# GEOS-ESM/GEOSradiation_GridComp

Measured on AMD Instinct MI355X. Metric: columns/sec (LW+SW, 72 layers), higher is better.
Workload: dtype f32; 1 GPU; BASELINE configs[3] (C360 tile / 8 GPUs) per-GPU share: 97200 columns/GPU, 72 layers, RRTMG_LW (140 g-points) + RRTMG_SW (112 g-points), McICA clouds on 60 % of the columns (ih=1), aerosols on, every column lit; schemes=RRTMG_LW (140 g-points) + RRTMG_SW (112 g-points), columns_per_gpu=97200, layers=72, aerosol=True, hip_streams=2

## Files before the change

geosradiation_gridcomp_amd/csrc/geosrad.hip:

```cpp
#include <hip/hip_runtime.h>

#include <cstdio>
#include <cstdlib>
#include <cstring>
#include <map>
#include <string>
#include <tuple>
#include <vector>
#include <thread>
#include <mutex>
#include <condition_variable>
#include <memory>
#include <atomic>
#include <functional>
#include <chrono>

#include <dlfcn.h>
#include <sched.h>
#include <cstddef>
#include <cstdint>
#include "../../include/geosrad.h"
#include "../../include/geosrad_gettau.h"
#include "../../include/geosrad_satsim.h"
#include "../../include/geosrad_misr_modis.h"
// ... 728 lines not shown
static inline ArrShape ic_in_shape(int k, size_t L) { return {k == geosrad_ctx::IC_PHALF ? L + 1 : k == geosrad_ctx::IC_SKT ? 1 : L, 1}; }
static inline ArrShape ic_out_shape(int k, size_t S) { return {k == geosrad_ctx::ICO_FQ ? 49 : k >= geosrad_ctx::ICO_BOXTAU ? S : 1, 1}; }
static inline ArrShape modis_in_shape(int k, size_t L, size_t S) { return {k == geosrad_ctx::MDI_PH ? L + 1 : k >= geosrad_ctx::MDI_BOXTAU ? S : L, 1}; }
static inline ArrShape modis_out_shape(int k, size_t S) { return {k == geosrad_ctx::MDO_MEAN ? (size_t)17 : k == geosrad_ctx::MDO_HIST ? (size_t)49 : S, 1}; }
static inline ArrShape misr_out_shape(int k) { return {k == geosrad_ctx::MIO_FQ ? (size_t)(7 * 16) : k == geosrad_ctx::MIO_DIST ? (size_t)16 : (size_t)1, 1}; }

struct HostArrs {
    size_t E;
    std::vector<geosrad_ctx::PipeArr> arrs;
    std::vector<const void **> at;
    explicit HostArrs(size_t real_bytes) : E(real_bytes) {}
    void add(const void *src, void *dst, ArrShape s, const void **at_, size_t ebytes = 0)
    {
        arrs.push_back({src, dst, s.rows, s.rec * (ebytes ? ebytes : E), 0});
        at.push_back(at_);
    }
    void add(const void *src, void *dst, ArrShape s, void **at_, size_t ebytes = 0) { add(src, dst, s, (const void **)at_, ebytes); }
    void add_clear_counts(int32_t *dst, void **at_) { add(nullptr, dst, {4, 1}, at_, sizeof(int32_t)); }
};

geosrad_ctx *geosrad_new_ctx_f32();
geosrad_ctx *geosrad_new_ctx_f64();

#if !defined(GEOSRAD_PART) || GEOSRAD_PART != 0
namespace {

#define LAUNCH_WIDE(kernel, wide, ncol, rows, st, arg) do {                                                            \
        if (wide) hipLaunchKernelGGL((kernel<R, VW>), dim3(grid256((ncol) / VW), rows), dim3(256), 0, st, arg);       \
        else hipLaunchKernelGGL((kernel<R, 1>), dim3(grid256(ncol), rows), dim3(256), 0, st, arg); } while (0)
template <typename R> struct Ctx : geosrad_ctx {
    using R2 = typename Vec2<R>::T;
    DevBuf<> d_tab, d_xcw;
    size_t so_lds_set = 0;
    LwDev<R> h_T{};
    DevBuf<LwDev<R>> d_T;
    bool have_lw = false;
    DevBuf<> d_tab_sw;
    SwDev<R> h_S{};
    std::vector<R> avgcyc_mg, avgcyc_sb;
    DevBuf<SwDev<R>> d_S;
    bool have_sw = false;
    DevBuf<> d_ws_sw; int ws_sw_ncol = 0, ws_sw_nlay = 0, ws_sw_planes = 0; bool ws_sw_radval = false;
    DevBuf<> d_tab_so;
    SoradDev<R> h_O{};
    DevBuf<SoradDev<R>> d_O;
    bool have_sorad = false;
// ... 287 lines not shown
        if constexpr (SW) {
            hipLaunchKernelGGL(k_sw_validate<R>, dim3(gx), blk, 0, st, A);
        } else hipLaunchKernelGGL(k_validate_pwv<R>, dim3(gx), blk, 0, st, A, d_T);
        launch_partition(st, A.ncol, A.colcloudy, A.perm, A.nclear);
        span_end(st);
        span_begin(SW ? 7 : 1, st);
        if constexpr (SW) hipLaunchKernelGGL(k_sw_setcoef<R>, dim3(gx, A.nlay), blk, 0, st, A, dS);
        else hipLaunchKernelGGL((k_setcoef<R, true>), dim3(gx, A.nlay), blk, 0, st, A, d_T);
        span_end(st);
        span_begin(2, st);
        hipLaunchKernelGGL(k_overlap<R>, dim3(gx, A.nlay), blk, 0, st, A.ncol, A.ld, A.nlay, A.doy, A.zm, A.alat, (const int32_t *)A.perm,
                           (const int32_t *)A.nclear, dT, A.alpha, A.rcorr, A.laycloudy);
        span_end(st);
        McArgs<R> M{};
        M.ncol = A.ncol; M.ld = A.ld; M.nlay = A.nlay; M.nsubcol = SW ? NG_SW : NG_LW; M.doy = A.doy; M.cloudLM = A.cloudLM; M.cloudMH = A.cloudMH;
        M.iceflg = A.iceflg; M.liqflg = A.liqflg;
        for (int k = 0; k < 4; k++) M.so[k] = SW ? 4 - k : 1 + k;
        M.cwp_tiny = (R)1.e-20;
        M.play = A.play; M.ciwp = A.ciwp; M.clwp = A.clwp; M.rei = A.rei; M.rel = A.rel;
        M.alpha = A.alpha; M.rcorr = A.rcorr; M.perm = A.perm; M.nclear = A.nclear; M.cftop = A.colcloudy;
        M.taucmc = A.taucmc; M.laycloudy = A.laycloudy; M.clearCounts = A.clearCounts; M.err = A.err;
        if constexpr (SW) { M.cldf = A.cld; M.ssacmc = A.ssacmc; M.asmcmc = A.asmcmc; M.cotsum = A.cotsum; M.rvsum = rvsum; }
        else M.cldf = A.cldf;
        McPlan MP; int nseg = 0;
        if (const int rc = mc_plan(MODE, M.nsubcol, A.nlay, MP, nseg)) return rc;
        const dim3 grid(xcd_grid(A.ncol, 64, nseg));
        span_begin(3, st);
        if constexpr (SW) {
            if (radval) hipLaunchKernelGGL((k_mcica<R, 2, true>), grid, dim3(64), 0, st, M, MP, dT, dS);
            else hipLaunchKernelGGL((k_mcica<R, 2>), grid, dim3(64), 0, st, M, MP, dT, dS);
        } else hipLaunchKernelGGL((k_mcica<R, 0>), grid, dim3(64), 0, st, M, MP, dT, dS);
        span_end(st);
        return GEOSRAD_OK;
    }

    int lw_sweeps(hipStream_t st, const LwArgs<R> &A, const LwOut<R> &O, bool allow_cols)
    {
        const dim3 blk(256);
        const unsigned gx = grid256(A.ncol);
        const size_t lds = lw_bands_lds_bytes<R>();
        const bool cols = lw_cols_path && allow_cols;
        LwArgs<R> S = A;
        if (O.part_alt) S.part = const_cast<R *>(O.part_alt);
        span_begin(4, st);
        if (cols) {
            if (const int rc = hip_rc("lw_cols_launch", lw_cols_launch<R>(st, S, O, h_T, A.dbg_taug != nullptr))) return rc;
// ... 957 lines not shown
    size_t ws_layout_sw(int nc, int nlay, SwArgs<R> &w, R *&rvsum, Carve c, int planes, bool radval) const
    {
        const size_t cl = (size_t)nlay * nc;
        w.sc = c.take<R>(SW_NFIELD * cl);
        w.scidx = c.take<uint32_t>(cl);
        w.colcloudy = c.take<uint8_t>(nc);
        w.perm = c.take<int32_t>(nc);
        w.nclear = c.take<int32_t>(1 + part_blocks(nc));
        w.laycloudy = c.take<uint8_t>(cl);
        w.alpha = c.take<R>(cl);
        w.rcorr = c.take<R>(cl);
        w.taucmc = c.take<R>(NG_SW * cl);
        w.ssacmc = c.take<R>(NG_SW * cl);
        w.asmcmc = c.take<R>(NG_SW * cl);
        w.cotsum = c.take<R>((size_t)3 * NG_SW * nc);
        w.cell = c.take<R>((size_t)planes * NG_SW * nlay * (((size_t)nc + 255) & ~(size_t)255));
        const size_t slots = sw_path == 2 ? (size_t)(sw_reform_nslot<R>() > NB_SW ? sw_reform_nslot<R>() : NB_SW) : (size_t)NB_SW;
        w.part = c.take<R>((size_t)4 * slots * (nlay + 1) * nc);
        w.bsfc = c.take<R>((size_t)3 * slots * nc);
        w.cot = c.take<R>((size_t)8 * 6 * nc);
        rvsum = radval ? c.take<R>((size_t)3 * RV_NSUM * RV_NPAR * nc) : nullptr;
        return c.off;
    }
    int sw_planes(bool dbg) const { return (sw_path == 2 && !dbg) ? (sizeof(R) == 4 ? 5 : 15) : 14; }
    int ensure_ws_sw(int nc, int nlay, int planes, bool radval)
    {
        if (d_ws_sw && nc <= ws_sw_ncol && nlay == ws_sw_nlay && planes <= ws_sw_planes && (ws_sw_radval || !radval)) return GEOSRAD_OK;
        if (planes < ws_sw_planes) planes = ws_sw_planes;
        radval = radval || ws_sw_radval;
        const int want = (d_ws_sw && nlay == ws_sw_nlay && nc < ws_sw_ncol) ? ws_sw_ncol : nc;
        SwArgs<R> w; R *rvsum;
        const size_t need = ws_layout_sw(want, nlay, w, rvsum, Carve(), planes, radval);
        if (d_ws_sw.resize(need) != hipSuccess) return fail(GEOSRAD_ENOMEM, "hipMalloc of the SW workspace failed (" + std::to_string(need >> 20) +
                                                         " MiB); lower it with geosrad_set_chunk()");
        ws_sw_ncol = want; ws_sw_nlay = nlay; ws_sw_planes = planes; ws_sw_radval = radval;
        return GEOSRAD_OK;
    }

    static bool nrl_adjust(R solcycfr, const R *indsolvar, R *scl)
    {
        const R fmin = (R)0.0189, fmax = (R)0.3750, dmin2max = fmax - fmin, dmax2min = (R)1. - dmin2max;
        if (solcycfr >= 0 && solcycfr < fmin) {
            const R wgt = (solcycfr + (R)1. - fmax) / dmax2min;
            scl[0] = indsolvar[0] + wgt * ((R)1. - indsolvar[0]); scl[1] = indsolvar[1] + wgt * ((R)1. - indsolvar[1]);
        } else if (solcycfr >= fmin && solcycfr <= fmax) {
            const R wgt = (solcycfr - fmin) / dmin2max;
            scl[0] = (R)1. + wgt * (indsolvar[0] - (R)1.); scl[1] = (R)1. + wgt * (indsolvar[1] - (R)1.);
// ... 134 lines not shown
        return GEOSRAD_OK;
    }
    int sw_check_arrays(const void *const *in, void *const *out, int iaer, int do_drfband)
    {
        for (int k = 0; k < S_NIN; k++)
            if (!in[k] && !((k == S_TAUAER || k == S_SSAAER || k == S_ASMAER) && iaer != 10)) return fail(GEOSRAD_EINVAL, "null input array");
        for (int k = 0; k < SO_DRBAND; k++) if (!out[k]) return fail(GEOSRAD_EINVAL, "null output array");
        if (do_drfband && (!out[SO_DRBAND] || !out[SO_DFBAND])) return fail(GEOSRAD_EINVAL, "do_drfband set but drband/dfband null");
        return GEOSRAD_OK;
    }

    int sw_run(hipStream_t st, int ncol, int nlay, double scon, double adjes, int isolvar, const void *const *in, int iceflg, int liqflg,
               int dyofyr, int iaer, int cloudLM, int cloudMH, int normFlx, int32_t *clearCounts, void *const *out, int do_drfband,
               const void *bndscl, const void *indsolvar, const void *solcycfrac, void *const *dbg, void *const *sw_na_out,
               void *radval = nullptr)
    {
        HIPCHK(hipSetDevice(device));
        if (const int rc = sw_check_options(ncol, nlay, iceflg, liqflg, cloudLM, cloudMH, iaer)) return rc;
        if (const int rc = sw_check_arrays(in, out, iaer, do_drfband)) return rc;
        if (radval && dbg) return fail(GEOSRAD_EINVAL, "the stage dumps do not produce the SOLAR_RADVAL diagnostics");
        SwSolar<R> SV;
        if (const int rc = sw_solar(scon, adjes, isolvar, (const R *)bndscl, (const R *)indsolvar, (const R *)solcycfrac, SV)) return rc;

        const int nc_max = chunk_cols(ncol, (long)(0xFFFFFFFFull / ((unsigned long long)nlay * 12ull * sizeof(R))) & ~255L);
        if (const int rc = ensure_ws_sw(nc_max, nlay, sw_planes(dbg != nullptr), radval != nullptr)) return rc;

        return chunk_walk(ncol, nc_max, [&](int c0, int nc) -> int {
            SwArgs<R> A{};
            R *rvsum;
            ws_layout_sw(nc, nlay, A, rvsum, Carve(d_ws_sw), ws_sw_planes, ws_sw_radval);
            A.ncol = nc; A.ld = ncol; A.nlay = nlay; A.iceflg = iceflg; A.liqflg = liqflg; A.doy = dyofyr; A.cloudLM = cloudLM;
            A.cloudMH = cloudMH; A.iaer = iaer; A.normFlx = normFlx; A.do_drfband = do_drfband;
            auto P = [&](int k) { return colp(in[k], c0); };
            A.play = P(S_PLAY); A.plev = P(S_PLEV); A.tlay = P(S_TLAY); A.h2o = P(S_H2O); A.o3 = P(S_O3); A.co2 = P(S_CO2);
            A.ch4 = P(S_CH4); A.o2 = P(S_O2); A.cld = P(S_CLD); A.ciwp = P(S_CIWP); A.clwp = P(S_CLWP); A.rei = P(S_REI);
            A.rel = P(S_REL); A.zm = P(S_ZM); A.alat = P(S_ALAT);
            A.tauaer = iaer == 10 ? P(S_TAUAER) : nullptr; A.ssaaer = iaer == 10 ? P(S_SSAAER) : nullptr;
            A.asmaer = iaer == 10 ? P(S_ASMAER) : nullptr;
            A.coszen = P(S_COSZEN); A.asdir = P(S_ASDIR); A.asdif = P(S_ASDIF); A.aldir = P(S_ALDIR); A.aldif = P(S_ALDIF);
            A.err = d_err + 1;
            A.clearCounts = clearCounts + c0;
            const size_t d0 = (size_t)c0 * NG_SW * nlay;
            if (dbg) { A.dbg_taug = (R *)dbg[0] + d0; A.dbg_taur = (R *)dbg[1] + d0; A.dbg_ssi = (R *)dbg[2] + (size_t)c0 * NG_SW; }
            if (const int e = rrtmg_front<2>(st, A, radval != nullptr, rvsum)) return e;
            const dim3 blk(256);
            const unsigned gx = grid256(nc);
            if (radval) {
// ... 1788 lines not shown

static __global__ void k_dbg_fast64(int n, const double *__restrict__ a, const double *__restrict__ b, double *__restrict__ q,
                                    double *__restrict__ r, double *__restrict__ s)
{
    const int i = blockIdx.x * blockDim.x + threadIdx.x;
    if (i < n) { q[i] = geosrad::gr_div64(a[i], b[i]); r[i] = geosrad::gr_rcp64(b[i]); s[i] = geosrad::gr_sqrt64(b[i]); }
}
int geosrad_dbg_fast64(int n, const double *a, const double *b, double *quot, double *rcp, double *root)
{
    if (n <= 0 || !a || !b || !quot || !rcp || !root) return GEOSRAD_EINVAL;
    DevBuf<double> d;
    const size_t nb = (size_t)n * sizeof(double);
    if (d.resize(5 * nb) != hipSuccess) return GEOSRAD_EHIP;
    int rc = GEOSRAD_OK;
    if (hipMemcpy(d, a, nb, hipMemcpyHostToDevice) != hipSuccess || hipMemcpy(d + n, b, nb, hipMemcpyHostToDevice) != hipSuccess) rc = GEOSRAD_EHIP;
    if (rc == GEOSRAD_OK) {
        k_dbg_fast64<<<(n + 255) / 256, 256>>>(n, d, d + n, d + 2 * (size_t)n, d + 3 * (size_t)n, d + 4 * (size_t)n);
        if (hipMemcpy(quot, d + 2 * (size_t)n, nb, hipMemcpyDeviceToHost) != hipSuccess || hipMemcpy(rcp, d + 3 * (size_t)n, nb, hipMemcpyDeviceToHost) != hipSuccess ||
            hipMemcpy(root, d + 4 * (size_t)n, nb, hipMemcpyDeviceToHost) != hipSuccess) rc = GEOSRAD_EHIP;
    }
    return rc;
}

int geosrad_rrtmg_lw_taumol(geosrad_ctx *c, int ncol, int nlay, const void *play, const void *plev, const void *tlay, const void *tlev,
                            const void *tsfc, const void *emis, const void *h2ovmr, const void *o3vmr, const void *co2vmr,
                            const void *ch4vmr, const void *n2ovmr, const void *o2vmr, const void *cfc11vmr, const void *cfc12vmr,
                            const void *cfc22vmr, const void *ccl4vmr, const void *tauaer, void *taug, void *pfracs)
{
    if (!c || !taug || !pfracs) return GEOSRAD_EINVAL;
    const size_t esz = (size_t)c->real_kind;
    std::vector<char> zero((size_t)ncol * (nlay + 1) * esz, 0), ones((size_t)ncol * nlay * esz, 0), scratch((size_t)ncol * (nlay + 1) * esz * 4);
    for (size_t i = 0; i < (size_t)ncol * nlay; i++) { if (esz == 4) ((float *)ones.data())[i] = 10.f; else ((double *)ones.data())[i] = 10.; }
    std::vector<int32_t> cc((size_t)ncol * 4);
    const void *cldf = zero.data(), *ciwp = zero.data(), *clwp = zero.data(), *rei = ones.data(), *rel = ones.data(), *zm = zero.data(),
               *alat = zero.data();
    LW_PACK_IN();
    char *s = scratch.data();
    const size_t cv = (size_t)ncol * (nlay + 1) * esz;
    void *out[O_NOUT] = {s, s + cv, s + 2 * cv, s + 3 * cv, nullptr, nullptr, nullptr, nullptr};
    return c->lw_host(ncol, nlay, 0, in, 3, 1, 1, 1, 2, cc.data(), out, nullptr, taug, pfracs);
}

int geosrad_mcica(geosrad_ctx *c, int ncol, int nsubcol, int nlay, const void *zmid, const void *alat, int doy, const void *play,
                  const void *cldfrac, const void *ciwp, const void *clwp, double cwp_tiny, const int32_t seed_order[4],
                  int32_t *cldy_stoch, void *ciwp_stoch, void *clwp_stoch)
{
// ... 36 lines not shown
```

geosradiation_gridcomp_amd/csrc/lw_kernels.hpp:

```cpp
#pragma once
#include "lw_device.hpp"
#include <type_traits>

namespace geosrad {

#define GR_DEV __device__ __forceinline__

template <typename R> GR_DEV R gr_exp(R x);
template <> GR_DEV float gr_exp<float>(float x) { return expf(x); }
template <> GR_DEV double gr_exp<double>(double x) { return exp(x); }
template <typename R> GR_DEV R gr_log(R x);
template <> GR_DEV float gr_log<float>(float x) { return logf(x); }
template <> GR_DEV double gr_log<double>(double x) { return log(x); }
template <typename R> GR_DEV R gr_log10(R x);
template <> GR_DEV float gr_log10<float>(float x) { return log10f(x); }
template <> GR_DEV double gr_log10<double>(double x) { return log10(x); }
template <typename R> GR_DEV R gr_pow(R x, R y);
template <> GR_DEV float gr_pow<float>(float x, float y) { return powf(x, y); }
template <> GR_DEV double gr_pow<double>(double x, double y) { return pow(x, y); }

#ifndef GR_FAST64
#define GR_FAST64 1
#endif
GR_DEV double gr_rcp64(double b)
// ... 21 lines not shown
    if (x == 0.0) return 0.0;
    const double y = __builtin_amdgcn_rsq(x);
    double g = x * y, h = 0.5 * y;
    const double r = fma(-h, g, 0.5);
    g = fma(g, r, g); h = fma(h, r, h);
    g = fma(fma(-g, g, x), h, g);
    return fma(fma(-g, g, x), h, g);
#else
    return sqrt(x);
#endif
}

GR_DEV int clampi(int v, int lo, int hi) { return v < lo ? lo : (v > hi ? hi : v); }

constexpr int pad4(int n) { return (n + 3) & ~3; }

template <typename T> GR_DEV T ldg(const T *base, uint32_t byteoff)
{
    return *reinterpret_cast<const T *>(reinterpret_cast<const char *>(base) + byteoff);
}
template <typename T> GR_DEV void stg(T *base, uint32_t byteoff, T v)
{
    *reinterpret_cast<T *>(reinterpret_cast<char *>(base) + byteoff) = v;
}
template <typename T> GR_DEV T ldg_nt(const T *base, uint32_t byteoff)
{
    return __builtin_nontemporal_load(reinterpret_cast<const T *>(reinterpret_cast<const char *>(base) + byteoff));
}
template <typename T> GR_DEV void stg_nt(T *base, uint32_t byteoff, T v)
{
    __builtin_nontemporal_store(v, reinterpret_cast<T *>(reinterpret_cast<char *>(base) + byteoff));
}
GR_DEV void err_wave(bool bad, uint32_t *err, int bit)
{
    if (__ballot(bad) != 0) {
        if (bad) atomicOr(err, 1u << bit);
    }
}
typedef float gr_v2f __attribute__((ext_vector_type(2)));
typedef double gr_v2d __attribute__((ext_vector_type(2)));
template <> GR_DEV float2 ldg_nt<float2>(const float2 *base, uint32_t byteoff)
{
    const gr_v2f t = __builtin_nontemporal_load(reinterpret_cast<const gr_v2f *>(reinterpret_cast<const char *>(base) + byteoff));
    float2 r; r.x = t.x; r.y = t.y; return r;
}
template <> GR_DEV double2 ldg_nt<double2>(const double2 *base, uint32_t byteoff)
// ... 1255 lines not shown
        BAND::template prep<R>(T, A, L, P);
#pragma unroll
        for (int q = 0; q < NQ; q++) {
            R tau[W], pf[W];
            BAND::template eval<R, W>(T, L, P, q * W, tau, pf);
#pragma unroll
            for (int j = 0; j < W; j++) {
                const int g = q * W + j;
                if (g >= NG) continue;
                if (lay == 0) {
                    const R rad0 = pf[j] * plankbnd;
                    rad[g] = rad0 + reflect * rad[g];
                    dlu[g] = pf[j] * dplankbnd;
                    u0 = u0 + sumfac * rad[g];
                    du0 = du0 + sumfac * dlu[g];
                    if (CLD) {
                        radc[g] = rad0 + reflect * radc[g];
                        dclu[g] = dlu[g];
                        uc0 = uc0 + sumfac * radc[g];
                        duc0 = duc0 + sumfac * dclu[g];
                    }
                }
                const R2 e1 = lut_at((int)sv[g]);
                const R a1 = (R)1. - e1.x, b1 = pf[j] * (blay + e1.y * dplankup);
                rad[g] = rad[g] + (b1 - rad[g]) * a1;
                dlu[g] = dlu[g] - dlu[g] * a1;
                usum = usum + sumfac * rad[g];
                dusum = dusum + sumfac * dlu[g];
                if (CLD) {
                    const R2 e2 = lut_at(own ? (int)sg[g] : (int)sv[g]);
                    const R gx = (R)1. - e2.x, gy = pf[j] * (blay + e2.y * dplankup);
                    const R rc = radc[g] + (gy - radc[g]) * gx, dc = dclu[g] - dclu[g] * gx;
                    radc[g] = diverge ? rc : rad[g];
                    dclu[g] = diverge ? dc : dlu[g];
                    ucsum = ucsum + sumfac * radc[g];
                    ducsum = ducsum + sumfac * dclu[g];
                }
            }
        }
        if (lay == 0) {
            PART(2, 0, u0);
            if (CLD && ccol) PART(3, 0, uc0);
            if (dudTs) { PART(4, 0, du0); if (CLD && ccol) PART(5, 0, duc0); }
        }
        PART(2, lay + 1, usum);
        if (CLD && ccol) PART(3, lay + 1, ucsum);
        if (dudTs) { PART(4, lay + 1, dusum); if (CLD && ccol) PART(5, lay + 1, ducsum); }
    }
#undef PART
}

__constant__ const int LW_BAND_ORDER[NB_LW] = {3, 5, 4, 7, 9, 2, 1, 8, 12, 6, 11, 13, 10, 15, 16, 14};
__host__ __device__ constexpr int lw_band_g0(int ib)
{
// ... 140 lines not shown
```

geosradiation_gridcomp_amd/csrc/sw_kernels.hpp:

```cpp
#pragma once
#include "lw_kernels.hpp"

namespace geosrad {

constexpr int NB_SW = 14;
constexpr int NG_SW = 112;

enum SwGas { G_H2O = 0, G_CO2, G_O3, G_CH4, G_O2, G_NONE };
enum SwScField {
    SW_FAC00 = 0, SW_FAC01, SW_FAC10, SW_FAC11, SW_COLH2O, SW_COLCO2, SW_COLO3, SW_COLCH4, SW_COLO2, SW_COLMOL,
    SW_SELFFAC, SW_SELFFRAC, SW_FORFAC, SW_FORFRAC, SW_NFIELD
};

template <typename R> struct SwBandTab {
    const R *absa, *absb, *selfref, *forref;
    const R *sflux, *irrad, *facb, *snsp;
    const R *rayl;
    const R *x0, *x1;
    const R *raylb;
};

template <typename R> struct SwDev {
    SwBandTab<R> b[NB_SW + 1];
    const R *preflog, *tref;
// ... 120 lines not shown
    A.scidx[(size_t)lay * n + col] = pack_idx(jp, jt, jt1, indfor, indself, 0, lower ? 1 : 0);
}

struct SwB16 { static constexpr int JB = 16, NG = 6,  G0 = 0,   LOK = 2, LOA = G_H2O, LOB = G_CH4, UPK = 1, UPA = G_CH4, UPB = G_NONE, NFOR = 3, SRC = 0, LREF = 0,  NSRC = 1; static constexpr double STR = 252.131;    static constexpr bool LOCONT = true,  UPFOR = false; };
struct SwB17 { static constexpr int JB = 17, NG = 12, G0 = 6,   LOK = 2, LOA = G_H2O, LOB = G_CO2, UPK = 2, UPA = G_H2O, UPB = G_CO2,  NFOR = 4, SRC = 2, LREF = 30, NSRC = 5; static constexpr double STR = 0.364641;   static constexpr bool LOCONT = true,  UPFOR = true;  };
struct SwB18 { static constexpr int JB = 18, NG = 8,  G0 = 18,  LOK = 2, LOA = G_H2O, LOB = G_CH4, UPK = 1, UPA = G_CH4, UPB = G_NONE, NFOR = 3, SRC = 1, LREF = 6,  NSRC = 9; static constexpr double STR = 38.9589;    static constexpr bool LOCONT = true,  UPFOR = false; };
struct SwB19 { static constexpr int JB = 19, NG = 8,  G0 = 26,  LOK = 2, LOA = G_H2O, LOB = G_CO2, UPK = 1, UPA = G_CO2, UPB = G_NONE, NFOR = 3, SRC = 1, LREF = 3,  NSRC = 9; static constexpr double STR = 5.49281;    static constexpr bool LOCONT = true,  UPFOR = false; };
struct SwB20 { static constexpr int JB = 20, NG = 10, G0 = 34,  LOK = 1, LOA = G_H2O, LOB = G_NONE, UPK = 1, UPA = G_H2O, UPB = G_NONE, NFOR = 4, SRC = 0, LREF = 0,  NSRC = 1; static constexpr double STR = 0;          static constexpr bool LOCONT = true,  UPFOR = true;  };
struct SwB21 { static constexpr int JB = 21, NG = 10, G0 = 44,  LOK = 2, LOA = G_H2O, LOB = G_CO2, UPK = 2, UPA = G_H2O, UPB = G_CO2,  NFOR = 4, SRC = 1, LREF = 8,  NSRC = 9; static constexpr double STR = 0.0045321;  static constexpr bool LOCONT = true,  UPFOR = true;  };
struct SwB22 { static constexpr int JB = 22, NG = 2,  G0 = 54,  LOK = 2, LOA = G_H2O, LOB = G_O2,  UPK = 1, UPA = G_O2,  UPB = G_NONE, NFOR = 3, SRC = 1, LREF = 2,  NSRC = 9; static constexpr double STR = 1.6 * 0.022708; static constexpr bool LOCONT = true, UPFOR = false; };
struct SwB23 { static constexpr int JB = 23, NG = 10, G0 = 56,  LOK = 1, LOA = G_H2O, LOB = G_NONE, UPK = 0, UPA = G_NONE, UPB = G_NONE, NFOR = 3, SRC = 0, LREF = 0,  NSRC = 1; static constexpr double STR = 0;          static constexpr bool LOCONT = true,  UPFOR = false; };
struct SwB24 { static constexpr int JB = 24, NG = 8,  G0 = 66,  LOK = 2, LOA = G_H2O, LOB = G_O2,  UPK = 1, UPA = G_O2,  UPB = G_NONE, NFOR = 3, SRC = 1, LREF = 1,  NSRC = 9; static constexpr double STR = 0.124692;   static constexpr bool LOCONT = true,  UPFOR = false; };
struct SwB25 { static constexpr int JB = 25, NG = 6,  G0 = 74,  LOK = 1, LOA = G_H2O, LOB = G_NONE, UPK = 0, UPA = G_NONE, UPB = G_NONE, NFOR = 0, SRC = 0, LREF = 0,  NSRC = 1; static constexpr double STR = 0;          static constexpr bool LOCONT = false, UPFOR = false; };
struct SwB26 { static constexpr int JB = 26, NG = 6,  G0 = 80,  LOK = 0, LOA = G_NONE, LOB = G_NONE, UPK = 0, UPA = G_NONE, UPB = G_NONE, NFOR = 0, SRC = 0, LREF = 0,  NSRC = 1; static constexpr double STR = 0;         static constexpr bool LOCONT = false, UPFOR = false; };
struct SwB27 { static constexpr int JB = 27, NG = 8,  G0 = 86,  LOK = 1, LOA = G_O3,  LOB = G_NONE, UPK = 1, UPA = G_O3,  UPB = G_NONE, NFOR = 0, SRC = 0, LREF = 0,  NSRC = 1; static constexpr double STR = 0;          static constexpr bool LOCONT = false, UPFOR = false; };
struct SwB28 { static constexpr int JB = 28, NG = 6,  G0 = 94,  LOK = 2, LOA = G_O3,  LOB = G_O2,  UPK = 2, UPA = G_O3,  UPB = G_O2,   NFOR = 0, SRC = 2, LREF = 42, NSRC = 5; static constexpr double STR = 6.67029e-07; static constexpr bool LOCONT = false, UPFOR = false; };
struct SwB29 { static constexpr int JB = 29, NG = 12, G0 = 100, LOK = 1, LOA = G_H2O, LOB = G_NONE, UPK = 1, UPA = G_CO2, UPB = G_NONE, NFOR = 4, SRC = 0, LREF = 0,  NSRC = 1; static constexpr double STR = 0;          static constexpr bool LOCONT = true,  UPFOR = false; };

template <typename R> struct SwLayer {
    R fac00, fac01, fac10, fac11, col[5], colmol, selffac, selffrac, forfac, forfrac;
    int jp, jt, jt1, indfor, indself;
    bool lower;
};
template <typename R> GR_DEV void sw_load_layer(const SwArgs<R> &A, int lay, int col, SwLayer<R> &L)
{
    const uint32_t cell = (uint32_t)lay * (uint32_t)A.ncol + (uint32_t)col;
    const uint32_t wb = cell * (uint32_t)sizeof(R);
    const size_t fs = (size_t)A.nlay * A.ncol;
#define SCF(f) ldg(A.sc + (size_t)(f) * fs, wb)
    L.fac00 = SCF(SW_FAC00); L.fac01 = SCF(SW_FAC01); L.fac10 = SCF(SW_FAC10); L.fac11 = SCF(SW_FAC11);
    L.col[G_H2O] = SCF(SW_COLH2O); L.col[G_CO2] = SCF(SW_COLCO2); L.col[G_O3] = SCF(SW_COLO3); L.col[G_CH4] = SCF(SW_COLCH4);
    L.col[G_O2] = SCF(SW_COLO2); L.colmol = SCF(SW_COLMOL);
    L.selffac = SCF(SW_SELFFAC); L.selffrac = SCF(SW_SELFFRAC); L.forfac = SCF(SW_FORFAC); L.forfrac = SCF(SW_FORFRAC);
#undef SCF
    const uint32_t p = ldg(A.scidx, cell * 4u);
    L.jp = p & 63; L.jt = (p >> 6) & 7; L.jt1 = (p >> 9) & 7; L.indfor = (p >> 12) & 3; L.indself = (p >> 14) & 15;
    L.lower = (p >> 23) & 1;
}

template <typename R> struct SwSpec { R speccomb, fs; int js; };
template <typename R> GR_DEV SwSpec<R> sw_spec(R cola, R strrat, R colb, R mult, R oneminus)
{
    SwSpec<R> s;
    s.speccomb = cola + strrat * colb;
    R specparm = cola / s.speccomb;
    if (specparm >= oneminus) specparm = oneminus;
    const R sm = mult * specparm;
    const int j = (int)sm;
    s.js = 1 + j;
    s.fs = sm - (R)j;
    return s;
}

template <typename R> struct SwPrep { SwSpec<R> sp; int ind0, ind1; R cmaj, extra; };

template <typename R, typename B> GR_DEV void sw_prep(const SwDev<R> &T, const SwLayer<R> &L, SwPrep<R> &P)
{
    P.extra = 0; P.cmaj = 0; P.ind0 = 1; P.ind1 = 1; P.sp.fs = 0; P.sp.js = 1; P.sp.speccomb = 0;
    if (L.lower) {
        if constexpr (B::LOK == 2) {
            P.sp = sw_spec<R>(L.col[B::LOA], (R)B::STR, L.col[B::LOB], 8, T.oneminus);
// ... 690 lines not shown
```

geosradiation_gridcomp_amd/csrc/sw_reform.hip:

```cpp
#include "sw_reform_kernels.hpp"
#include "sw_reform.hpp"

namespace geosrad {

template <typename R> hipError_t sw_reform_launch(hipStream_t st, const SwArgs<R> &A, const SwDev<R> &T, const SwSolar<R> &SV)
{
    static_assert(swr_nslot<R> <= SWR_SLOTS_MAX && swr_ncot<R> <= 6, "workspace slots");
    const dim3 grid(band_grid(A.ncol, swr_nslot<R>)), blk(256);
    hipLaunchKernelGGL((k_sw_reform<R, false>), grid, blk, 0, st, A, T, SV);
    hipLaunchKernelGGL((k_sw_reform<R, true>), grid, blk, 0, st, A, T, SV);
    return hipGetLastError();
}

template <typename R> int sw_reform_nslot() { return swr_nslot<R>; }

template <typename R> int sw_reform_par_units(int *sizes)
{
    int k = 0;
    for (int jb = 24; jb <= 26; jb++)
        for (int u = 0; u < swr_nunit(swr_u<R>, sw_band_ng(jb)); u++) sizes[k++] = swr_usize(swr_u<R>, sw_band_ng(jb), u);
    return k;
}

template <typename R> hipError_t sw_reform_reduce(hipStream_t st, const SwArgs<R> &A, const SwOut<R> &O)
{
    hipLaunchKernelGGL(k_swr_reduce<R>, dim3((unsigned)((A.ncol + 255) / 256), A.nlay + 2), dim3(256), 0, st, A, O);
    return hipGetLastError();
}

#if !defined(GEOSRAD_PART) || GEOSRAD_PART == 4
template hipError_t sw_reform_launch<float>(hipStream_t, const SwArgs<float> &, const SwDev<float> &, const SwSolar<float> &);
template hipError_t sw_reform_reduce<float>(hipStream_t, const SwArgs<float> &, const SwOut<float> &);
template int sw_reform_nslot<float>();
template int sw_reform_par_units<float>(int *);
#endif
#if !defined(GEOSRAD_PART) || GEOSRAD_PART == 8
template hipError_t sw_reform_launch<double>(hipStream_t, const SwArgs<double> &, const SwDev<double> &, const SwSolar<double> &);
template hipError_t sw_reform_reduce<double>(hipStream_t, const SwArgs<double> &, const SwOut<double> &);
template int sw_reform_nslot<double>();
template int sw_reform_par_units<double>(int *);
#endif

}
```

geosradiation_gridcomp_amd/csrc/sw_reform.hpp:

```cpp
#pragma once
#include "sw_kernels.hpp"

namespace geosrad {
constexpr int SWR_SLOTS_MAX = 32;
template <typename R> int sw_reform_nslot();
template <typename R> int sw_reform_par_units(int *sizes);
template <typename R> hipError_t sw_reform_launch(hipStream_t st, const SwArgs<R> &A, const SwDev<R> &T, const SwSolar<R> &SV);
template <typename R> hipError_t sw_reform_reduce(hipStream_t st, const SwArgs<R> &A, const SwOut<R> &O);
}
```

geosradiation_gridcomp_amd/csrc/sw_reform_kernels.hpp:

```cpp
#pragma once
#include "sw_kernels.hpp"

namespace geosrad {

template <typename B> struct SwrRaylPerG { static constexpr bool value = B::JB >= 23 && B::JB <= 27; };

#ifndef SWR_U
#define SWR_U 6
#endif
#ifndef SWR_U64
#define SWR_U64 4
#endif
template <typename R> constexpr int swr_u = sizeof(R) == 8 ? SWR_U64 : SWR_U;
__host__ __device__ constexpr int swr_nunit(int U, int ng) { return (ng + U - 1) / U; }
__host__ __device__ constexpr int swr_usize(int U, int ng, int u)
{
    const int nu = swr_nunit(U, ng);
    if (nu == 1) return ng;
    const int pairs = ng / 2, base = pairs / nu, extra = pairs % nu;
    return 2 * (base + (u < extra ? 1 : 0));
}
__host__ __device__ constexpr int swr_ustart(int U, int ng, int u) { int s = 0; for (int k = 0; k < u; k++) s += swr_usize(U, ng, k); return s; }
__host__ __device__ constexpr int swr_slot0(int U, int jb) { int s = 0; for (int b = 16; b < jb; b++) s += swr_nunit(U, sw_band_ng(b)); return s; }
template <typename R> constexpr int swr_nslot = swr_slot0(swr_u<R>, 30);
// ... 61 lines not shown
        for (int q = 0; q < NQ; q++) {
            R sf[W], fb[W], sd[W], ir[W];
            const int go = GO + q * W;
            if constexpr (B::NSRC == 1) {
                ldw<R, W>(Bt.sflux, (uint32_t)go * (uint32_t)sizeof(R), sf); ldw<R, W>(Bt.facb, (uint32_t)go * (uint32_t)sizeof(R), fb);
                ldw<R, W>(Bt.snsp, (uint32_t)go * (uint32_t)sizeof(R), sd); ldw<R, W>(Bt.irrad, (uint32_t)go * (uint32_t)sizeof(R), ir);
            } else {
                linw<R, W, S>(sf, fs, Bt.sflux, js - 1, go); linw<R, W, S>(fb, fs, Bt.facb, js - 1, go);
                linw<R, W, S>(sd, fs, Bt.snsp, js - 1, go); linw<R, W, S>(ir, fs, Bt.irrad, js - 1, go);
            }
#pragma unroll
            for (int j = 0; j < W; j++) {
                const int g = q * W + j;
                if (g >= NG) continue;
                R src;
                if (SV.isolvar < 0) src = sf[j];
                else if (SV.isolvar <= 2) src = SV.svar_f * fb[j] + SV.svar_s * sd[j] + SV.svar_i * ir[j];
                else src = SV.svar_bnd[IBM] * fb[j] + SV.svar_bnd[IBM] * sd[j] + SV.svar_bnd[IBM] * ir[j];
                zinc[g] = SV.adjflux[IBM] * src;
            }
        }
    }

    const uint32_t npad = ((uint32_t)n + 255u) & ~255u;
    const size_t plane = (size_t)NG_SW * nlay * npad;
    R *const cellb = A.cell + (size_t)G0 * nlay * npad;
    const uint32_t tbase = (ucol >> 8) * (uint32_t)nlay * (uint32_t)NGB * 256u + (ucol & 255u);
    const size_t bandoff = (size_t)G0 * nlay * n;
    const R *const tcb = A.taucmc + bandoff, *const ocb = A.ssacmc + bandoff, *const gcb = A.asmcmc + bandoff;
#define CELL(q) (cellb + (size_t)(q) * plane)
#define PST(q, off, v) stg_nt(CELL(q), off, v)
#define PLD(q, off) ldg_nt(CELL(q), off)
#define CT4(lay_, g_) ((tbase + ((uint32_t)(lay_) * (uint32_t)NGB + (uint32_t)(GO + (g_))) * 256u) * (uint32_t)sizeof(R))
#define MC4(lay_, g_) ((((uint32_t)(lay_) * (uint32_t)NGB + (uint32_t)(GO + (g_))) * (uint32_t)n + ucol) * (uint32_t)sizeof(R))
    const size_t aerb = (size_t)(IBM - 1) * nlay * ld;

    R prup[NG], prupd[NG], prupT[NG], prupdT[NG];
    int lowc[NG];
#pragma unroll
    for (int g = 0; g < NG; g++) { prup[g] = albp; prupd[g] = albd; prupT[g] = albp; prupdT[g] = albd; lowc[g] = 0x7fffffff; }
    int lcA = CLD ? (int)ldg(A.laycloudy, ucol) : 0;
#pragma nounroll
    for (int lay = 0; lay < nlay; lay++) {
        const int lcA_cur = lcA;
        if (CLD && lay + 1 < nlay) lcA = (int)ldg(A.laycloudy, (uint32_t)(lay + 1) * (uint32_t)n + ucol);
        SwLayer<R> L;
        sw_load_layer<R>(A, lay, col, L);
        R ta = 0, om = 1, as = 0;
        if (A.iaer == 10) {
            const uint32_t ab = ((uint32_t)lay * (uint32_t)ld + (uint32_t)pc) * (uint32_t)sizeof(R);
            ta = ldg(A.tauaer + aerb, ab); om = ldg(A.ssaaer + aerb, ab); as = ldg(A.asmaer + aerb, ab);
        }
        const bool laycld = CLD && ccol && lcA_cur != 0;
        const bool wlc = CLD && __ballot(laycld) != 0;
        SwPrep<R> P;
        sw_prep<R, B>(T, L, P);
        R tr0 = 0;
#pragma unroll
        for (int q = 0; q < NQ; q++) {
            R tcv[W], ocv[W], gcv[W];
#pragma unroll
            for (int j = 0; j < W; j++) { tcv[j] = 0; ocv[j] = 0; gcv[j] = 0; }
            if (wlc) {
#pragma unroll
                for (int j = 0; j < W; j++)
                    if (q * W + j < NG) {
                        tcv[j] = ldg(tcb, MC4(lay, q * W + j));
                        ocv[j] = ldg(ocb, MC4(lay, q * W + j)); gcv[j] = ldg(gcb, MC4(lay, q * W + j));
                    }
            }
// ... 31 lines not shown
                    if (ccol && !divg) { prupT[g] = prup[g]; prupdT[g] = prupd[g]; }
                    if (divg) {
                        SwCell<R> t = c;
                        if (cellcld) {
                            sw_cell_cloud<R>(c, tcv[j], ocv[j], gcv[j], prmu0, rmu0, t);
                            if constexpr (!REFORM) { PST(10, ct4, t.ref); PST(11, ct4, t.refd); PST(12, ct4, t.tra); PST(13, ct4, t.trad); PST(14, ct4, t.dbt); }
                        }
                        const R zrj = f_rcp<R>((R)1. - prupdT[g] * t.refd);
                        const R pu = t.ref + (t.trad * ((t.tra - t.dbt) * prupdT[g] + t.dbt * prupT[g])) * zrj;
                        const R pd = t.refd + t.trad * t.trad * prupdT[g] * zrj;
                        prupT[g] = pu; prupdT[g] = pd;
                        PST(3, ct4, pu); PST(4, ct4, pd);
                    }
                }
            }
#ifndef SWR_NO_GROUP_BARRIER
            __builtin_amdgcn_sched_barrier(0);
#endif
        }
        sw_assert_aer<R>(A, ta, om);
    }

    const size_t qs = (size_t)swr_nslot<R> * (nlay + 1) * n;
    R *const part = A.part + (size_t)SLOT * (nlay + 1) * n;
#ifdef SWR_PART_NT
#define PART(kind, lev, val) stg_nt(part + (size_t)(kind) * qs + (size_t)(lev) * n, cb, (R)(val))
#else
#define PART(kind, lev, val) stg(part + (size_t)(kind) * qs + (size_t)(lev) * n, cb, (R)(val))
#endif
    R tdbt[NG], ztdn[NG], prdnd[NG], tdbtT[NG], ztdnT[NG], prdndT[NG];
    uint32_t dmask = 0;
    {
        R cu = 0, cd = 0, fu = 0, fd = 0;
#pragma unroll
        for (int g = 0; g < NG; g++) {
            tdbt[g] = 1; ztdn[g] = 1; prdnd[g] = 0; tdbtT[g] = 1; ztdnT[g] = 1; prdndT[g] = 0;
            const R zi = zinc[g] * prmu0;
            {
                const R pu = prup[g], pd = prupd[g];
                const R zr = f_rcp<R>((R)1. - prdnd[g] * pd);
                cu = cu + zi * ((tdbt[g] * pu + (ztdn[g] - tdbt[g]) * pd) * zr);
                cd = cd + zi * (tdbt[g] + (ztdn[g] - tdbt[g] + tdbt[g] * pu * prdnd[g]) * zr);
            }
            if (CLD && ccol) {
                const R puT = prupT[g], pdT = prupdT[g];
                const R zr = f_rcp<R>((R)1. - prdndT[g] * pdT);
                fu = fu + zi * ((tdbtT[g] * puT + (ztdnT[g] - tdbtT[g]) * pdT) * zr);
// ... 16 lines not shown
            else { for (int k = 0; k < 5; k++) b.lp[k][j] = PLD(5 + k, CT4(lay, g)); }
            b.pu[j] = PLD(1, CT4(lu, g)); b.pd[j] = PLD(2, CT4(lu, g));
        }
    };
    struct Lay { R colmol, ta, om, as; uint32_t idx; R ca, cb2; };
    auto request_layer = [&](int lay, Lay &b) {
        const uint32_t wb = ((uint32_t)lay * (uint32_t)n + ucol) * (uint32_t)sizeof(R);
        const size_t fs_ = (size_t)nlay * n;
        b.colmol = ldg(A.sc + (size_t)SW_COLMOL * fs_, wb);
        b.ta = 0; b.om = 1; b.as = 0; b.idx = 0; b.ca = 0; b.cb2 = 0;
        if (A.iaer == 10) {
            const uint32_t ab = ((uint32_t)lay * (uint32_t)ld + (uint32_t)pc) * (uint32_t)sizeof(R);
            b.ta = ldg(A.tauaer + aerb, ab); b.om = ldg(A.ssaaer + aerb, ab); b.as = ldg(A.asmaer + aerb, ab);
        }
        if constexpr (B::JB == 24) {
            b.idx = ldg(A.scidx, ((uint32_t)lay * (uint32_t)n + ucol) * 4u);
            b.ca = ldg(A.sc + (size_t)(SW_COLH2O + B::LOA) * fs_, wb); b.cb2 = ldg(A.sc + (size_t)(SW_COLH2O + B::LOB) * fs_, wb);
        }
    };
    Park nx; Lay nl;
    request_layer(nlay - 1, nl);
    request(nlay - 1, 0, nx);
    R sdir = 0, sfd = 0, sfu = 0;
    int lcB = CLD ? (int)ldg(A.laycloudy, (uint32_t)(nlay - 1) * (uint32_t)n + ucol) : 0;
#pragma nounroll
    for (int lay = nlay - 1; lay >= 0; lay--) {
        const int lcB_cur = lcB;
        if (CLD && lay > 0) lcB = (int)ldg(A.laycloudy, (uint32_t)(lay - 1) * (uint32_t)n + ucol);
        const int jk = nlay - 1 - lay;
        const Lay cl = nl;
        request_layer(lay > 0 ? lay - 1 : 0, nl);
        const bool laycld = CLD && ccol && lcB_cur != 0;
        const bool wlc = CLD && __ballot(laycld) != 0;
        bool lower = true; int js = 1; R fs = 0;
        if constexpr (B::JB == 24) {
            lower = (cl.idx >> 23) & 1u;
            const SwSpec<R> sp = sw_spec<R>(cl.ca, (R)B::STR, cl.cb2, 8, T.oneminus);
            js = sp.js; fs = sp.fs;
        }
        R tr0 = 0;
        R cu = 0, cd = 0, fu = 0, fd = 0;
#pragma unroll
        for (int q = 0; q < NQ; q++) {
            Park cur = nx;
            if (q + 1 < NQ) request(lay, q + 1, nx);
            else request(lay > 0 ? lay - 1 : 0, 0, nx);
            R tcv[W], ocv[W], gcv[W], puT[W], pdT[W];
            bool dv[W], anydv = false;
#pragma unroll
            for (int j = 0; j < W; j++) {
                const int g = q * W + j;
// ... 253 lines not shown
```

Before: 5.398 million columns/s.

## Interleave SW parked planes in 5-plane groups and pin base pointers in SGPRs

Stores the SW reform kernel's parked per-cell planes as interleaved groups of five planes with a 256-element stride, so one column's planes sit close together. Base pointers are kept in scalar registers through an empty asm barrier, and the field stride is computed once with readfirstlane, which is meant to cut address arithmetic and VGPR pressure. In the LW cloudy sweep, the second LUT lookup is skipped for layers above the cloud top. The change also adds 32-bit offset bound checks and a debug query entry point, which can reject some chunk sizes that were accepted before.

New measurement: 5.407 million columns/s (median of 2 runs). No clear change (+0.2%).

```diff
diff --git a/geosradiation_gridcomp_amd/csrc/geosrad.hip b/geosradiation_gridcomp_amd/csrc/geosrad.hip
--- a/geosradiation_gridcomp_amd/csrc/geosrad.hip
+++ b/geosradiation_gridcomp_amd/csrc/geosrad.hip
@@ -774,6 +774,13 @@
 geosrad_ctx *geosrad_new_ctx_f32();
 geosrad_ctx *geosrad_new_ctx_f64();
 
+static inline bool band_plane_offsets_fit(long ncol, long nlay, int max_ng, size_t elem)
+{
+    if (ncol <= 0 || nlay <= 0) return false;
+    const unsigned long long per = (unsigned long long)nlay * (unsigned long long)max_ng * elem;
+    return (unsigned long long)ncol <= 0xFFFFFFFFull / per;
+}
+
 #if !defined(GEOSRAD_PART) || GEOSRAD_PART != 0
 namespace {
 
@@ -1107,6 +1114,8 @@
         M.taucmc = A.taucmc; M.laycloudy = A.laycloudy; M.clearCounts = A.clearCounts; M.err = A.err;
         if constexpr (SW) { M.cldf = A.cld; M.ssacmc = A.ssacmc; M.asmcmc = A.asmcmc; M.cotsum = A.cotsum; M.rvsum = rvsum; }
         else M.cldf = A.cldf;
+        if (!band_plane_offsets_fit(A.ncol, A.nlay, SW ? 12 : 16, SW ? sizeof(R) : sizeof(R2)))
+            return fail(GEOSRAD_EINVAL, "RRTMG: a band's per-cell plane exceeds 32-bit byte offsets; lower the chunk with geosrad_set_chunk()");
         McPlan MP; int nseg = 0;
         if (const int rc = mc_plan(MODE, M.nsubcol, A.nlay, MP, nseg)) return rc;
         const dim3 grid(xcd_grid(A.ncol, 64, nseg));
@@ -2110,7 +2119,7 @@
         rvsum = radval ? c.take<R>((size_t)3 * RV_NSUM * RV_NPAR * nc) : nullptr;
         return c.off;
     }
-    int sw_planes(bool dbg) const { return (sw_path == 2 && !dbg) ? (sizeof(R) == 4 ? 5 : 15) : 14; }
+    int sw_planes(bool dbg) const { return (sw_path == 2 && !dbg) ? swr_nplane<R> : 14; }
     int ensure_ws_sw(int nc, int nlay, int planes, bool radval)
     {
         if (d_ws_sw && nc <= ws_sw_ncol && nlay == ws_sw_nlay && planes <= ws_sw_planes && (ws_sw_radval || !radval)) return GEOSRAD_OK;
@@ -2291,7 +2300,11 @@
         SwSolar<R> SV;
         if (const int rc = sw_solar(scon, adjes, isolvar, (const R *)bndscl, (const R *)indsolvar, (const R *)solcycfrac, SV)) return rc;
 
-        const int nc_max = chunk_cols(ncol, (long)(0xFFFFFFFFull / ((unsigned long long)nlay * 12ull * sizeof(R))) & ~255L);
+        const bool reform_cells = sw_reform_on() && !dbg;
+        static_assert(SW_NFIELD <= 12 * SWR_PG, "the parked planes' bound covers the setcoef record");
+        const int nc_max = chunk_cols(ncol, (long)(0xFFFFFFFFull / ((unsigned long long)nlay * (reform_cells ? 12ull * SWR_PG : (unsigned long long)SW_NFIELD) * sizeof(R))) & ~255L);
+        if (reform_cells && !sw_reform_offsets_fit<R>(nc_max, nlay))
+            return fail(GEOSRAD_EINVAL, "RRTMG_SW: a band's parked planes exceed 32-bit byte offsets; lower the chunk with geosrad_set_chunk()");
         if (const int rc = ensure_ws_sw(nc_max, nlay, sw_planes(dbg != nullptr), radval != nullptr)) return rc;
 
         return chunk_walk(ncol, nc_max, [&](int c0, int nc) -> int {
@@ -4126,6 +4139,16 @@
     return rc;
 }
 
+extern "C" int geosrad_dbg_band_offsets(int real_kind, int solver, long ncol, long nlay)
+{
+    if ((real_kind != 4 && real_kind != 8) || (solver != 0 && solver != 2)) return GEOSRAD_EINVAL;
+    bool ok;
+    if (solver == 0) ok = band_plane_offsets_fit(ncol, nlay, 16, 2 * (size_t)real_kind);
+    else ok = band_plane_offsets_fit(ncol, nlay, 12, (size_t)real_kind) &&
+              (real_kind == 4 ? geosrad::sw_reform_offsets_fit<float>(ncol, nlay) : geosrad::sw_reform_offsets_fit<double>(ncol, nlay));
+    return ok ? GEOSRAD_OK : GEOSRAD_EINVAL;
+}
+
 int geosrad_rrtmg_lw_taumol(geosrad_ctx *c, int ncol, int nlay, const void *play, const void *plev, const void *tlay, const void *tlev,
                             const void *tsfc, const void *emis, const void *h2ovmr, const void *o3vmr, const void *co2vmr,
                             const void *ch4vmr, const void *n2ovmr, const void *o2vmr, const void *cfc11vmr, const void *cfc12vmr,
diff --git a/geosradiation_gridcomp_amd/csrc/lw_kernels.hpp b/geosradiation_gridcomp_amd/csrc/lw_kernels.hpp
--- a/geosradiation_gridcomp_amd/csrc/lw_kernels.hpp
+++ b/geosradiation_gridcomp_amd/csrc/lw_kernels.hpp
@@ -67,6 +67,13 @@
 template <typename T> GR_DEV void stg(T *base, uint32_t byteoff, T v)
 {
     *reinterpret_cast<T *>(reinterpret_cast<char *>(base) + byteoff) = v;
+}
+template <typename T> GR_DEV T *gr_own(T *p)
+{
+    typedef T __attribute__((address_space(1))) *gT;
+    gT a = (gT)p;
+    asm volatile("" : "+s"(a));
+    return (T *)a;
 }
 template <typename T> GR_DEV T ldg_nt(const T *base, uint32_t byteoff)
 {
@@ -1368,14 +1375,19 @@
                     }
                 }
                 const R2 e1 = lut_at((int)sv[g]);
-                const R a1 = (R)1. - e1.x, b1 = pf[j] * (blay + e1.y * dplankup);
+                const R x1 = blay + e1.y * dplankup;
+                const R a1 = (R)1. - e1.x, b1 = pf[j] * x1;
                 rad[g] = rad[g] + (b1 - rad[g]) * a1;
                 dlu[g] = dlu[g] - dlu[g] * a1;
                 usum = usum + sumfac * rad[g];
                 dusum = dusum + sumfac * dlu[g];
                 if (CLD) {
-                    const R2 e2 = lut_at(own ? (int)sg[g] : (int)sv[g]);
-                    const R gx = (R)1. - e2.x, gy = pf[j] * (blay + e2.y * dplankup);
+                    R gx = a1, xg = x1;
+                    if (lay <= wtop) {
+                        const R2 e2 = lut_at(own ? (int)sg[g] : (int)sv[g]);
+                        gx = (R)1. - e2.x; xg = blay + e2.y * dplankup;
+                    }
+                    const R gy = pf[j] * xg;
                     const R rc = radc[g] + (gy - radc[g]) * gx, dc = dclu[g] - dclu[g] * gx;
                     radc[g] = diverge ? rc : rad[g];
                     dclu[g] = diverge ? dc : dlu[g];
diff --git a/geosradiation_gridcomp_amd/csrc/sw_kernels.hpp b/geosradiation_gridcomp_amd/csrc/sw_kernels.hpp
--- a/geosradiation_gridcomp_amd/csrc/sw_kernels.hpp
+++ b/geosradiation_gridcomp_amd/csrc/sw_kernels.hpp
@@ -166,12 +166,18 @@
     int jp, jt, jt1, indfor, indself;
     bool lower;
 };
-template <typename R> GR_DEV void sw_load_layer(const SwArgs<R> &A, int lay, int col, SwLayer<R> &L)
+template <typename R> GR_DEV uint32_t sw_field_bytes(const SwArgs<R> &A) { return (uint32_t)A.nlay * (uint32_t)A.ncol * (uint32_t)sizeof(R); }
+template <typename R> GR_DEV uint32_t sw_field_bytes_in_loop(const SwArgs<R> &A)
+{
+    uint32_t fsb = (uint32_t)__builtin_amdgcn_readfirstlane((int)sw_field_bytes<R>(A));
+    asm volatile("" : "+s"(fsb));
+    return fsb;
+}
+template <typename R> GR_DEV void sw_load_layer(const SwArgs<R> &A, int lay, int col, SwLayer<R> &L, uint32_t fsb)
 {
     const uint32_t cell = (uint32_t)lay * (uint32_t)A.ncol + (uint32_t)col;
     const uint32_t wb = cell * (uint32_t)sizeof(R);
-    const size_t fs = (size_t)A.nlay * A.ncol;
-#define SCF(f) ldg(A.sc + (size_t)(f) * fs, wb)
+#define SCF(f) ldg(reinterpret_cast<const R *>(reinterpret_cast<const char *>(A.sc) + (size_t)((uint32_t)(f) * fsb)), wb)
     L.fac00 = SCF(SW_FAC00); L.fac01 = SCF(SW_FAC01); L.fac10 = SCF(SW_FAC10); L.fac11 = SCF(SW_FAC11);
     L.col[G_H2O] = SCF(SW_COLH2O); L.col[G_CO2] = SCF(SW_COLCO2); L.col[G_O3] = SCF(SW_COLO3); L.col[G_CH4] = SCF(SW_COLCH4);
     L.col[G_O2] = SCF(SW_COLO2); L.colmol = SCF(SW_COLMOL);
@@ -181,6 +187,7 @@
     L.jp = p & 63; L.jt = (p >> 6) & 7; L.jt1 = (p >> 9) & 7; L.indfor = (p >> 12) & 3; L.indself = (p >> 14) & 15;
     L.lower = (p >> 23) & 1;
 }
+template <typename R> GR_DEV void sw_load_layer(const SwArgs<R> &A, int lay, int col, SwLayer<R> &L) { sw_load_layer<R>(A, lay, col, L, sw_field_bytes<R>(A)); }
 
 template <typename R> struct SwSpec { R speccomb, fs; int js; };
 template <typename R> GR_DEV SwSpec<R> sw_spec(R cola, R strrat, R colb, R mult, R oneminus)
diff --git a/geosradiation_gridcomp_amd/csrc/sw_reform.hip b/geosradiation_gridcomp_amd/csrc/sw_reform.hip
--- a/geosradiation_gridcomp_amd/csrc/sw_reform.hip
+++ b/geosradiation_gridcomp_amd/csrc/sw_reform.hip
@@ -13,6 +13,17 @@
 }
 
 template <typename R> int sw_reform_nslot() { return swr_nslot<R>; }
+
+template <typename R> bool sw_reform_offsets_fit(long ncol, long nlay)
+{
+    if (ncol <= 0 || nlay <= 0) return false;
+    const unsigned long long n = (unsigned long long)ncol, npad = (n + 255ull) & ~255ull, l = (unsigned long long)nlay, lim = 0xFFFFFFFFull;
+    const unsigned long long tile = npad * l * 12ull * SWR_PG * sizeof(R);
+    const unsigned long long mc = n * l * 12ull * sizeof(R);
+    const unsigned long long sc = n * l * (unsigned long long)SW_NFIELD * sizeof(R);
+    if (sc > lim) return false;
+    return npad <= lim && tile / (12ull * SWR_PG * sizeof(R)) / l == npad && tile <= lim && mc <= lim;
+}
 
 template <typename R> int sw_reform_par_units(int *sizes)
 {
@@ -32,12 +43,14 @@
 template hipError_t sw_reform_launch<float>(hipStream_t, const SwArgs<float> &, const SwDev<float> &, const SwSolar<float> &);
 template hipError_t sw_reform_reduce<float>(hipStream_t, const SwArgs<float> &, const SwOut<float> &);
 template int sw_reform_nslot<float>();
+template bool sw_reform_offsets_fit<float>(long, long);
 template int sw_reform_par_units<float>(int *);
 #endif
 #if !defined(GEOSRAD_PART) || GEOSRAD_PART == 8
 template hipError_t sw_reform_launch<double>(hipStream_t, const SwArgs<double> &, const SwDev<double> &, const SwSolar<double> &);
 template hipError_t sw_reform_reduce<double>(hipStream_t, const SwArgs<double> &, const SwOut<double> &);
 template int sw_reform_nslot<double>();
+template bool sw_reform_offsets_fit<double>(long, long);
 template int sw_reform_par_units<double>(int *);
 #endif
 
diff --git a/geosradiation_gridcomp_amd/csrc/sw_reform.hpp b/geosradiation_gridcomp_amd/csrc/sw_reform.hpp
--- a/geosradiation_gridcomp_amd/csrc/sw_reform.hpp
+++ b/geosradiation_gridcomp_amd/csrc/sw_reform.hpp
@@ -4,6 +4,9 @@
 namespace geosrad {
 constexpr int SWR_SLOTS_MAX = 32;
 template <typename R> int sw_reform_nslot();
+constexpr int SWR_PG = 5;
+template <typename R> constexpr int swr_nplane = sizeof(R) == 4 ? SWR_PG : 3 * SWR_PG;
+template <typename R> bool sw_reform_offsets_fit(long ncol, long nlay);
 template <typename R> int sw_reform_par_units(int *sizes);
 template <typename R> hipError_t sw_reform_launch(hipStream_t st, const SwArgs<R> &A, const SwDev<R> &T, const SwSolar<R> &SV);
 template <typename R> hipError_t sw_reform_reduce(hipStream_t st, const SwArgs<R> &A, const SwOut<R> &O);
diff --git a/geosradiation_gridcomp_amd/csrc/sw_reform_kernels.hpp b/geosradiation_gridcomp_amd/csrc/sw_reform_kernels.hpp
--- a/geosradiation_gridcomp_amd/csrc/sw_reform_kernels.hpp
+++ b/geosradiation_gridcomp_amd/csrc/sw_reform_kernels.hpp
@@ -1,5 +1,6 @@
 #pragma once
 #include "sw_kernels.hpp"
+#include "sw_reform.hpp"
 
 namespace geosrad {
 
@@ -107,16 +108,18 @@
         }
     }
 
+    static_assert((REFORM ? 4 : 14) < swr_nplane<R> && swr_nplane<R> % SWR_PG == 0, "highest parked plane");
     const uint32_t npad = ((uint32_t)n + 255u) & ~255u;
-    const size_t plane = (size_t)NG_SW * nlay * npad;
-    R *const cellb = A.cell + (size_t)G0 * nlay * npad;
-    const uint32_t tbase = (ucol >> 8) * (uint32_t)nlay * (uint32_t)NGB * 256u + (ucol & 255u);
+    const size_t pgroup = (size_t)SWR_PG * NG_SW * nlay * npad;
+    R *const cellb = gr_own(A.cell + (size_t)SWR_PG * G0 * nlay * npad + (SWR_PG / 2) * 256);
+    const uint32_t tbase = (ucol >> 8) * (uint32_t)nlay * (uint32_t)NGB * (uint32_t)(SWR_PG * 256) + (ucol & 255u);
     const size_t bandoff = (size_t)G0 * nlay * n;
-    const R *const tcb = A.taucmc + bandoff, *const ocb = A.ssacmc + bandoff, *const gcb = A.asmcmc + bandoff;
-#define CELL(q) (cellb + (size_t)(q) * plane)
+    const R *const tcb = gr_own(A.taucmc + bandoff), *const ocb = gr_own(A.ssacmc + bandoff), *const gcb = gr_own(A.asmcmc + bandoff);
+    const uint8_t *const lcb = gr_own(A.laycloudy);
+#define CELL(q) (cellb + (size_t)((q) / SWR_PG) * pgroup + (((q) % SWR_PG) - SWR_PG / 2) * 256)
 #define PST(q, off, v) stg_nt(CELL(q), off, v)
 #define PLD(q, off) ldg_nt(CELL(q), off)
-#define CT4(lay_, g_) ((tbase + ((uint32_t)(lay_) * (uint32_t)NGB + (uint32_t)(GO + (g_))) * 256u) * (uint32_t)sizeof(R))
+#define CT4(lay_, g_) ((tbase + ((uint32_t)(lay_) * (uint32_t)NGB + (uint32_t)(GO + (g_))) * (uint32_t)(SWR_PG * 256)) * (uint32_t)sizeof(R))
 #define MC4(lay_, g_) ((((uint32_t)(lay_) * (uint32_t)NGB + (uint32_t)(GO + (g_))) * (uint32_t)n + ucol) * (uint32_t)sizeof(R))
     const size_t aerb = (size_t)(IBM - 1) * nlay * ld;
 
@@ -124,13 +127,13 @@
     int lowc[NG];
 #pragma unroll
     for (int g = 0; g < NG; g++) { prup[g] = albp; prupd[g] = albd; prupT[g] = albp; prupdT[g] = albd; lowc[g] = 0x7fffffff; }
-    int lcA = CLD ? (int)ldg(A.laycloudy, ucol) : 0;
+    int lcA = CLD ? (int)ldg(lcb, ucol) : 0;
 #pragma nounroll
     for (int lay = 0; lay < nlay; lay++) {
         const int lcA_cur = lcA;
-        if (CLD && lay + 1 < nlay) lcA = (int)ldg(A.laycloudy, (uint32_t)(lay + 1) * (uint32_t)n + ucol);
+        if (CLD && lay + 1 < nlay) lcA = (int)ldg(lcb, (uint32_t)(lay + 1) * (uint32_t)n + ucol);
         SwLayer<R> L;
-        sw_load_layer<R>(A, lay, col, L);
+        sw_load_layer<R>(A, lay, col, L, sw_field_bytes_in_loop<R>(A));
         R ta = 0, om = 1, as = 0;
         if (A.iaer == 10) {
             const uint32_t ab = ((uint32_t)lay * (uint32_t)ld + (uint32_t)pc) * (uint32_t)sizeof(R);
@@ -208,7 +211,7 @@
     }
 
     const size_t qs = (size_t)swr_nslot<R> * (nlay + 1) * n;
-    R *const part = A.part + (size_t)SLOT * (nlay + 1) * n;
+    R *const part = gr_own(A.part + (size_t)SLOT * (nlay + 1) * n);
 #ifdef SWR_PART_NT
 #define PART(kind, lev, val) stg_nt(part + (size_t)(kind) * qs + (size_t)(lev) * n, cb, (R)(val))
 #else
@@ -271,11 +274,11 @@
     request_layer(nlay - 1, nl);
     request(nlay - 1, 0, nx);
     R sdir = 0, sfd = 0, sfu = 0;
-    int lcB = CLD ? (int)ldg(A.laycloudy, (uint32_t)(nlay - 1) * (uint32_t)n + ucol) : 0;
+    int lcB = CLD ? (int)ldg(lcb, (uint32_t)(nlay - 1) * (uint32_t)n + ucol) : 0;
 #pragma nounroll
     for (int lay = nlay - 1; lay >= 0; lay--) {
         const int lcB_cur = lcB;
-        if (CLD && lay > 0) lcB = (int)ldg(A.laycloudy, (uint32_t)(lay - 1) * (uint32_t)n + ucol);
+        if (CLD && lay > 0) lcB = (int)ldg(lcb, (uint32_t)(lay - 1) * (uint32_t)n + ucol);
         const int jk = nlay - 1 - lay;
         const Lay cl = nl;
         request_layer(lay > 0 ? lay - 1 : 0, nl);
```
